# Lounes78/matcha-tts

Hardware: AMD Instinct MI355X
Metric: mel-frames/sec + RTF, text->wav @10 ODE steps, LJSpeech model, 1/2/4/8 GPU (higher is better)
Workload: dtype bf16

## Files before the change

include/matcha_hip.h:

```cpp
#ifndef MATCHA_HIP_H
#define MATCHA_HIP_H

#include <stddef.h>
#include <stdint.h>

#ifdef __cplusplus
extern "C" {
#endif

#define MT_DTYPE_F32 0
#define MT_DTYPE_BF16 1
#define MT_SOLVER_EULER 0
#define MT_SOLVER_MIDPOINT 1

const char* mt_last_error(void);
int mt_abi_version(void);
int mt_build_experiments(void);
int mt_sched_count(void);
int mt_sched_get(int i, int* rec, int* wait, int* wait_first, int cap);

typedef struct mt_encoder mt_encoder;
int mt_encoder_create(int n_vocab, int n_channels, int filter_channels, int n_heads, int n_layers, int kernel_size,
                      int n_spks, int spk_emb_dim, int dp_filter_channels, int dp_kernel_size, int prenet, int dtype,
                      mt_encoder** out);
// ... 176 lines not shown
                      int rows, int C, float* dx, void* stream);
int mtt_snake_fwd(const float* x, const float* log_alpha, const float* log_beta, size_t n, int C, float* y,
                  void* stream);
int mtt_snake_bwd(const float* x, const float* log_alpha, const float* log_beta, const float* dy, size_t n, int C,
                  float* dx, float* galpha, float* gbeta, void* stream);
int mtt_softmax_fwd(const float* s, const float* kmask, const float* qmask, int BH, int H, int Tq, int Tk, float scale,
                    int mode, float* p, void* stream);
int mtt_softmax_bwd(const float* p, const float* dp, const float* kmask, const float* qmask, int BH, int H, int Tq,
                    int Tk, float scale, float* ds, void* stream);
int mtt_rope(float* x, int B, int T, int H, int dh, int d, const float* theta, int inverse, void* stream);
int mtt_embed_fwd(const int64_t* ids, size_t ntok, const float* table, int C, float scale, float* out, void* stream);
int mtt_embed_bwd(const int64_t* ids, size_t ntok, const float* dout, int V, int C, float scale, float* dtable,
                  void* stream);
int mtt_adam(float* p, const float* g, float* m, float* v, size_t n, const float* gscale, float lr, float beta1,
             float beta2, float eps, int step, void* stream);
int mtt_clip_factor(const float* sumsq, float max_norm, float inv_world, float* out, float* norm_out, void* stream);
int mtt_unscale(float* g, size_t n, float inv_scale, float* found, float* scratch, void* stream);

size_t mt_op_conv1d_workspace_bytes(int dtype, int cin, int cout, int k, int stride, int transposed);
int mt_op_conv1d(int dtype, const void* x, int B, int Tin, int cin, const float* W, const float* bias,
                 int cout, int k, int stride, int pad, int dil, int transposed, float slope, void* y,
                 int Tout, void* ws, size_t ws_bytes, void* stream);
int mt_op_conv1d_tile(int variant, int dtype, const void* x, int B, int Tin, int cin, const float* W,
                      const float* bias, int cout, int k, int stride, int pad, int dil, int transposed,
                      float slope, void* y, int Tout, void* ws, size_t ws_bytes, void* stream);
size_t mt_op_vconv_workspace_bytes(int cin, int cout, int k);
int mt_op_vconv(const void* x, int B, int L, int cin, const float* W, const float* bias, int cout, int k, int dil,
                int ef, const void* resid, void* y, void* y2, float slope, float div, const int32_t* lens, int pack,
                void* ws, size_t ws_bytes, void* stream);
int mt_vconv_set_rbconv(int enable);
int mt_vconv_set_ct(int enable);
int mt_vpair_set_kernels(int mask);
int mt_vocoder_set_post_fold(int enable);
int mt_vconv_set_actin(int enable);
int mt_ffn_set(int enable);
int mt_ffn_set_min_frames(int frames);
int mt_decoder_set_kernels(int mask);
int mt_op_attention(int dtype, const void* qkv, const float* mask, void* out, int B, int T, int heads,
                    void* stream);

#define MT_PROBE_RBFUSE_C64 1
#define MT_PROBE_RBFUSE_C32 2
#define MT_PROBE_VCONV 3
#define MT_PROBE_VCONV_DEC 4
int mt_probe_start(int site, int max_launches);
int mt_probe_pause(int paused);
int mt_probe_detail(int cap, double* ms, double* flops, double* bytes, int* tags);
int mt_probe_stop(int* launches, double* total_ms, double* flops, double* bytes, double peak_flops, double peak_bw,
                  double* roof_ms);

#define MT_VCONV_LOG_FIELDS 11
int mt_vconv_log_start(int capacity);
int mt_vconv_log_stop(int32_t* records, int capacity);
int mt_vconv_log_select(int families);

#ifdef __cplusplus
}
#endif
#endif
```

matcha-tts_amd/csrc/mt_capi.hip:

```cpp
#include <string.h>

#include <new>

#include "../../include/matcha_hip.h"
#include "mt_ffn.h"
#include "mt_model.h"
#include "mt_vconv.h"
#include "mt_vpair.h"
#include "mt_probe.h"
#include "mt_train.h"

namespace mt {
const char* last_error();
int denoise(const float* audio, int B, int L, const float* bias_spec, float strength, float* out, void* ws,
            size_t ws_bytes, hipStream_t st, const int* lens = nullptr, int lmul = 1);
size_t denoise_workspace_bytes(int B, int L);
int vconv_exp_flags();
int rbconv_exp_flags();
int ffn_exp_flags();
int vpair_exp_flags();
int stft_magnitude(const float* audio, int B, int L, float* mag, hipStream_t st);
int log_mel(const float* audio, int B, int L, const float* basis, float mean, float stdv, float* mel, hipStream_t st);
size_t resample_workspace_bytes(int half, int up, int down);
int resample(const float* audio, int B, int L, const int* lens, int lmul, const float* taps, int half, int up,
// ... 19 lines not shown

struct mt_encoder {
  mt::Encoder e;
};
struct mt_decoder {
  mt::Decoder d;
};
struct mt_vocoder {
  mt::Vocoder v;
};

using mt::set_error;

static int param_name(const mt::ParamList& L, int i, char* buf, int buflen) {
  MT_REQUIRE(i >= 0 && i < (int)L.names.size(), "param index %d out of range", i);
  MT_REQUIRE(buf && buflen > (int)L.names[i].size(), "param name buffer too small");
  memcpy(buf, L.names[i].c_str(), L.names[i].size() + 1);
  return 0;
}
static int param_shape(const mt::ParamList& L, int i, int64_t* shape, int maxdim) {
  MT_REQUIRE(i >= 0 && i < (int)L.names.size(), "param index %d out of range", i);
  const auto& s = L.shapes[i];
  MT_REQUIRE((int)s.size() <= maxdim, "shape buffer too small");
  for (size_t k = 0; k < s.size(); ++k) shape[k] = s[k];
  return (int)s.size();
}

extern "C" {

const char* mt_last_error(void) { return mt::last_error(); }
int mt_abi_version(void) { return 1; }
int mt_vpair_set_kernels(int mask) { return mt::vpair_set_kernels(mask); }
int mt_vocoder_set_post_fold(int enable) { return mt::vocoder_set_post_fold(enable); }
int mt_sched_count(void) { return mt::sched_count(); }
int mt_sched_get(int i, int* rec, int* wait, int* wait_first, int cap) {
  MT_REQUIRE(rec && wait && wait_first, "null buffer");
  const int S = mt::sched_get(i, rec, wait, wait_first, cap);
  MT_REQUIRE(S >= 0, "schedule %d: out of range or cap %d too small", i, cap);
  return S;
}
int mt_build_experiments(void) {
  return (mt::vconv_exp_flags() ? 1 : 0) | (mt::rbconv_exp_flags() ? 2 : 0) | (mt::ffn_exp_flags() ? 4 : 0) |
         (mt::vpair_exp_flags() ? 8 : 0);
}

int mt_encoder_create(int n_vocab, int n_channels, int filter_channels, int n_heads, int n_layers, int kernel_size,
                      int n_spks, int spk_emb_dim, int dp_filter_channels, int dp_kernel_size, int prenet, int dtype,
                      mt_encoder** out) {
  MT_REQUIRE(out, "null out");
  mt_encoder* h = new (std::nothrow) mt_encoder();
  MT_REQUIRE(h, "out of host memory");
  int rc = h->e.init(n_vocab, n_channels, filter_channels, n_heads, n_layers, kernel_size, n_spks, spk_emb_dim,
                     dp_filter_channels, dp_kernel_size, prenet, dtype);
  if (rc) {
    delete h;
    return rc;
  }
  *out = h;
  return 0;
}
void mt_encoder_destroy(mt_encoder* e) { delete e; }
int mt_encoder_num_params(const mt_encoder* e) { return e ? (int)e->e.params.names.size() : -1; }
int mt_encoder_param_name(const mt_encoder* e, int i, char* buf, int buflen) {
  MT_REQUIRE(e, "null encoder");
  return param_name(e->e.params, i, buf, buflen);
}
// ... 609 lines not shown
```

matcha-tts_amd/csrc/mt_model.h:

```cpp
#pragma once
#include <memory>
#include <string>
#include <vector>

#include "mt_conv.h"
#include "mt_misc.h"
#include "mt_vconv.h"

namespace mt {

struct ParamList {
  std::vector<std::string> names;
  std::vector<std::vector<long long>> shapes;
  int add(const std::string& n, std::vector<long long> s) {
    names.push_back(n);
    shapes.push_back(std::move(s));
    return (int)names.size() - 1;
  }
};

struct Packer {
  size_t off = 0;
  size_t take(size_t bytes) {
    const size_t o = off;
// ... 160 lines not shown
  size_t emb_off = 0;
  struct Pre {
    GemmW conv;
    int g, b;
    size_t ln_off;
  };
  std::vector<Pre> pre;
  GemmW pre_proj;
  struct Layer {
    GemmW qkv, o, f1, f2;
    int n1g, n1b, n2g, n2b;
    size_t n1_off, n2_off;
    size_t s1_off = 0, s2_off = 0;
  };
  std::vector<Layer> lay;
  size_t ezero_off = 0;
  GemmW proj_m, dp1, dp2, dpp;
  int dn1g, dn1b, dn2g, dn2b, theta;
  size_t dn1_off, dn2_off, theta_off;

  int init(int n_vocab, int n_channels, int filter_channels, int heads, int layers, int kernel, int n_spks,
           int spk_dim, int dp_filter, int dp_kernel, int prenet, int dtype);
  int pack(const float* const* p, void* packed, hipStream_t st) const;
  size_t workspace_bytes(int B, int Tx) const;
  int forward(const void* packed, const long long* ids, const long long* xlen, const float* spks, int B, int Tx,
              float* mu, float* logw, float* xmask, int* oov, void* ws, size_t ws_bytes, hipStream_t st) const;
  template <class E>
  int forward_t(const char* P, const long long* ids, const long long* xlen, const float* spks, int B, int Tx,
                float* mu, float* logw, float* xmask, int* oov, char* ws, hipStream_t st) const;
};

int vocoder_post_fold();
int vocoder_set_post_fold(int enable);

struct Vocoder {
  int resblock = 1, dtype = BF16, esize = 2;
  int fuse = 1;
  int vconv = 2;
  int pair = 1;
  static constexpr int kDefaultWt = 0;
  int wt_stages = kDefaultWt;
  size_t zero_off = 0;
  bool any_vc = false;
  std::vector<int> up_rates, up_kernels, rb_kernels;
  std::vector<std::vector<int>> rb_dils;
  int up_init = 512, n_mels = 80;
  ParamList params;
  size_t packed_bytes = 0;
  GemmW pre, post;
  std::vector<GemmW> ups;
  std::vector<std::vector<GemmW>> rb1, rb2;

  int init(int resblock, const std::vector<int>& up_rates, const std::vector<int>& up_kernels, int up_init,
           const std::vector<int>& rb_kernels, const std::vector<std::vector<int>>& rb_dils, int dtype);
  int pack(const float* const* p, void* packed, hipStream_t st) const;
  bool stage_vc(int i) const;
  bool rb_vp(int i, int j) const;
  bool stage_vp(int i) const;
  bool stage_vp32(int i) const;
  int pair_resblock(const char* P, int i, int j, int B, int L, const char* X, char* XS, char* Tb, char* R,
                    char* RA, char* trash, bool act_out, hipStream_t st, const int* lens = nullptr,
                    float* wav = nullptr) const;
  int pair_chain(const char* P, int i, int B, int L, const char* X, char* XS, char* Tb, char* R, char* RA,
                 char* trash, bool act_out, hipStream_t st, const int* lens = nullptr, float* wav = nullptr) const;
  bool post_fold(int i) const;
  int rate_upto(int i) const;
// ... 18 lines not shown
```

matcha-tts_amd/csrc/mt_probe.cpp:

```cpp
#include "mt_probe.h"
#include "mt_vconv.h"

#include <algorithm>
#include <mutex>
#include <vector>

namespace mt {
namespace {
std::mutex g_mu;
int g_site = PROBE_NONE;
std::vector<hipEvent_t> g_ev;
int g_n = 0, g_cap = 0;
double g_flops = 0, g_bytes = 0;
std::vector<double> g_lf, g_lb;
std::vector<int> g_lt;
bool g_open = false;
bool g_paused = false;

void release() {
  for (hipEvent_t e : g_ev) (void)hipEventDestroy(e);
  g_ev.clear();
  g_n = g_cap = 0;
  g_flops = g_bytes = 0;
  g_lf.clear();
  g_lb.clear();
  g_lt.clear();
  g_site = PROBE_NONE;
  g_open = false;
  g_paused = false;
}
}

bool probe_armed(int site) { return g_site != PROBE_NONE && g_site == site; }
bool probe_any_armed() { return g_site != PROBE_NONE; }

void probe_begin(int site, hipStream_t st) {
  if (!probe_armed(site)) return;
  std::lock_guard<std::mutex> lk(g_mu);
  if (g_n >= g_cap || g_open || g_paused) return;
  (void)hipEventRecord(g_ev[2 * g_n], st);
  g_open = true;
}

void probe_end(int site, hipStream_t st, double flops, double bytes, int tag) {
  if (!probe_armed(site)) return;
  std::lock_guard<std::mutex> lk(g_mu);
  if (!g_open) return;
  (void)hipEventRecord(g_ev[2 * g_n + 1], st);
  g_open = false;
  ++g_n;
  g_flops += flops;
  g_bytes += bytes;
  g_lf.push_back(flops);
  g_lb.push_back(bytes);
  g_lt.push_back(tag);
}

int probe_detail(int cap, double* ms, double* flops, double* bytes, int* tags) {
  std::lock_guard<std::mutex> lk(g_mu);
  const int n = std::min(cap, g_n);
  for (int i = 0; i < n; ++i) {
    float t = 0.f;
    if (hipEventSynchronize(g_ev[2 * i + 1]) != hipSuccess ||
        hipEventElapsedTime(&t, g_ev[2 * i], g_ev[2 * i + 1]) != hipSuccess) {
      set_error("probe: event timing failed");
      return -1;
    }
    if (ms) ms[i] = t;
    if (flops) flops[i] = g_lf[i];
    if (bytes) bytes[i] = g_lb[i];
    if (tags) tags[i] = g_lt[i];
  }
  return n;
}

int probe_start(int site, int max_launches) {
  std::lock_guard<std::mutex> lk(g_mu);
  release();
  MT_REQUIRE(site > PROBE_NONE && site <= PROBE_VCONV_DEC, "probe: unknown site %d", site);
  MT_REQUIRE(max_launches > 0 && max_launches <= (1 << 16), "probe: max_launches %d", max_launches);
  g_ev.resize(2 * (size_t)max_launches);
  for (hipEvent_t& e : g_ev) MT_CHECK_HIP(hipEventCreate(&e));
  g_cap = max_launches;
  g_site = site;
  return 0;
}

int probe_pause(bool paused) {
  std::lock_guard<std::mutex> lk(g_mu);
  g_paused = paused;
  return 0;
}

int probe_stop(int* launches, double* total_ms, double* flops, double* bytes, double peak_flops, double peak_bw,
               double* roof_ms) {
  std::lock_guard<std::mutex> lk(g_mu);
  double ms = 0, roof = 0;
  for (int i = 0; i < g_n; ++i)
    roof += 1e3 * std::max(peak_flops > 0 ? g_lf[i] / peak_flops : 0.0, peak_bw > 0 ? g_lb[i] / peak_bw : 0.0);
  int rc = 0;
  for (int i = 0; i < g_n && rc == 0; ++i) {
    float t = 0.f;
    if (hipEventSynchronize(g_ev[2 * i + 1]) != hipSuccess ||
        hipEventElapsedTime(&t, g_ev[2 * i], g_ev[2 * i + 1]) != hipSuccess) {
      set_error("probe: event timing failed");
      rc = -1;
    }
    ms += t;
  }
  if (launches) *launches = g_n;
  if (total_ms) *total_ms = ms;
  if (flops) *flops = g_flops;
  if (bytes) *bytes = g_bytes;
  if (roof_ms) *roof_ms = roof;
  release();
  return rc;
}

namespace {
std::vector<int> g_log;
int g_log_cap = 0;
bool g_log_on = false;
}

namespace {
struct SchedEntry {
  int rec[SCHED_FIELDS];
  SchedWaits waits;
};
std::vector<SchedEntry>& sched_table() {
  static std::vector<SchedEntry> t;
  return t;
}
}

int sched_register(const int (&rec)[SCHED_FIELDS], SchedWaits waits) {
  auto& t = sched_table();
  for (const auto& e : t)
    if (std::equal(e.rec, e.rec + SCHED_FIELDS, rec)) return 0;
  SchedEntry e;
  std::copy(rec, rec + SCHED_FIELDS, e.rec);
  e.waits = waits;
  t.push_back(e);
// ... 49 lines not shown
```

matcha-tts_amd/csrc/mt_probe.h:

```cpp
#pragma once
#include "mt_common.h"

namespace mt {

enum ProbeSite {
  PROBE_NONE = 0,
  PROBE_RBFUSE_C64 = 1,
  PROBE_RBFUSE_C32 = 2,
  PROBE_VCONV = 3,
  PROBE_VCONV_DEC = 4,
};

bool probe_armed(int site);
bool probe_any_armed();
void probe_begin(int site, hipStream_t st);
enum ProbeTag { PROBE_TAG_VCONV = 0, PROBE_TAG_VPAIR = 1, PROBE_TAG_VPAIR32 = 2, PROBE_TAG_RBFUSE = 3, PROBE_TAG_VPAIR128 = 4, PROBE_TAG_RBCONV = 5 };
void probe_end(int site, hipStream_t st, double flops, double bytes, int tag = PROBE_TAG_VCONV);
int probe_detail(int cap, double* ms, double* flops, double* bytes, int* tags);
int probe_start(int site, int max_launches);
int probe_pause(bool paused);
int probe_stop(int* launches, double* total_ms, double* flops, double* bytes, double peak_flops, double peak_bw,
               double* roof_ms);

constexpr int VCLOG_FIELDS = 11;
enum : int { VCLOG_CONV = 1, VCLOG_AUX = 2 };
void vclog_record(const int (&rec)[VCLOG_FIELDS], int family = VCLOG_CONV);
int vclog_select(int families);
int vclog_start(int cap);
int vclog_stop(int* out, int cap);
bool vclog_armed();

}
```

matcha-tts_amd/csrc/mt_vocoder.hip:

```cpp
#include <algorithm>
#include <type_traits>

#include "mt_model.h"
#include "mt_ragged.h"
#include "mt_rbfuse.h"
#include "mt_vconv.h"
#include "mt_vpair.h"

namespace mt {

constexpr int PC_N = 256;
__global__ __launch_bounds__(256) void post_conv_kernel(const bf16* __restrict__ x, int L,
                                                        const bf16* __restrict__ w, const float* __restrict__ bias,
                                                        float slope, float* __restrict__ out, const int* lens,
                                                        int lmul) {
  __shared__ __attribute__((aligned(16))) char rows[(PC_N + 16) * 64];
  const int b = blockIdx.y, f0 = blockIdx.x * PC_N, tid = threadIdx.x, lane = tid & 63, wave = tid >> 6;
  const bf16* xb = x + (size_t)b * L * 32;
  const int Lb = lens ? min(max(lens[b] * lmul, 0), L) : L;
  if (f0 >= Lb) {
    if (f0 + tid < L) out[(size_t)b * L + f0 + tid] = 0.f;
    return;
  }
  for (int e = tid; e < (PC_N + 6) * 4; e += 256) {
// ... 215 lines not shown
}

bool Vocoder::stage_vp32(int i) const {
  const int nk = (int)rb_kernels.size();
  if (!pair || !fuse || vconv < 2 || !any_vc || dtype != BF16 || resblock != 1 || rb1[(size_t)i * nk].empty()) return false;
  for (int j = 0; j < nk; ++j)
    for (size_t q = 0; q < rb1[(size_t)i * nk + j].size(); ++q) {
      const GemmW& a = rb1[(size_t)i * nk + j][q];
      const GemmW& b = rb2[(size_t)i * nk + j][q];
      for (const GemmW* g : {&a, &b})
        if (g->cin != 32 || g->cout != 32 || g->Mpad != 32 || g->cin_pad != 32 || g->taps != g->k) return false;
      if (!vpair32_supported(a.k, a.dil) || b.k != a.k || b.dil != 1) return false;
    }
  return true;
}

static int g_postfold = -1;
int vocoder_post_fold() {
  if (g_postfold < 0) {
    const char* e = getenv("MT_POSTFOLD");
    g_postfold = e && e[0] == '0' ? 0 : 1;
  }
  return g_postfold;
}
int vocoder_set_post_fold(int enable) {
  const int prev = vocoder_post_fold();
  g_postfold = enable ? 1 : 0;
  return prev;
}

bool Vocoder::post_fold(int i) const {
  const int nk = (int)rb_kernels.size();
  return vocoder_post_fold() && dtype == BF16 && i + 1 == (int)ups.size() && stage_vp32(i) && post.cin == 32 &&
         post.k == 7 && post.cout == 1 && nk > 0 && (rb_kernels[nk - 1] - 1) / 2 <= 5;
}

int Vocoder::pair_resblock(const char* P, int i, int j, int B, int L, const char* X, char* XS, char* Tb, char* R,
                           char* RA, char* trash, bool act_out, hipStream_t st, const int* lens, float* wav) const {
  const int nk = (int)rb_kernels.size();
  const int C = rb1[(size_t)i * nk][0].cout;
  const bool c32 = C == 32;
  int rc;
  const std::vector<GemmW>& c1 = rb1[(size_t)i * nk + j];
  const std::vector<GemmW>& c2 = rb2[(size_t)i * nk + j];
  const int np = (int)c1.size();
  const char* state = X;
  for (int q = 0; q < np; ++q) {
    const bool last = q == np - 1;
    VPairArgs a{};
    a.x = (const bf16*)state;
    a.B = B;
    a.L = L;
    a.w1 = (const bf16*)(P + (c32 ? c1[q].w_off : c1[q].v_off));
    a.b1 = (const float*)(P + c1[q].b_off);
    a.w2 = (const bf16*)(P + (c32 ? c2[q].w_off : c2[q].v_off));
    a.b2 = (const float*)(P + c2[q].b_off);
    a.taps = c1[q].k;
    a.dil = c1[q].dil;
    a.div = (float)nk;
    a.slope = 0.1f;
    a.zero = (const bf16*)(P + zero_off);
    a.trash = (bf16*)trash;
    a.lens = lens;
    a.lmul = rate_upto(i + 1);
    int ef = 0;
    if (!last) {
      a.y = (bf16*)((q & 1) ? Tb : R);
    } else {
      a.y = (bf16*)XS;
      if (j > 0) ef |= VE_ACCUM;
      if (j == nk - 1) ef |= VE_DIV;
      if (j == nk - 1 && act_out) {
        a.y2 = (bf16*)RA;
        ef |= VE_DUAL | VE_Y2ONLY;
      }
      if (j == nk - 1 && wav && c32 && !act_out && j > 0) {
        a.post_w = (const bf16*)(P + post.w_off);
        a.post_b = (const float*)(P + post.b_off);
        a.post_slope = 0.01f;
// ... 371 lines not shown
```

matcha-tts_amd/csrc/mt_vpair.h:

```cpp
#pragma once
#include <algorithm>

#include "mt_probe.h"
#include "mt_ragged.h"
#include "mt_vconv.h"

namespace mt {

struct VPairArgs {
  const bf16* x;
  int B, L;
  const bf16* w1;
  const float* b1;
  const bf16* w2;
  const float* b2;
  int taps, dil;
  bf16* y;
  bf16* y2;
  float div, slope;
  const bf16* zero;
  bf16* trash;
  const int* lens;
  int lmul;
  const bf16* post_w;
// ... 156 lines not shown
      return (OPT & VE_POST) != 0;
  }
#undef MT_PAIR_EF
  return false;
}

template <class F>
int pair_launch(const char* name, int C, int bn, int ef, const VPairArgs& a, hipStream_t st, int tag, F&& launch) {
  const long ntiles = (long)a.B * ((a.L + bn - 1) / bn);
  MT_REQUIRE(ntiles < (1L << 31), "%s: too many tiles", name);
  const int G = (int)std::min<long>(ntiles, cu_count());
  const double flops = 2.0 * 2.0 * C * C * a.taps * (double)a.B * a.L;
  const double bytes = 2.0 * (2.0 * 2.0 * C * (double)a.B * a.L) + 2.0 * 2.0 * C * C * a.taps;
  probe_begin(PROBE_VCONV, st);
  if (!launch(G)) {
    set_error("%s: epilogue %d not compiled in", name, ef);
    return -1;
  }
  MT_CHECK_HIP(hipGetLastError());
  probe_end(PROBE_VCONV, st, flops, bytes, tag);
  const int rec[VCLOG_FIELDS] = {ef | 0x10000, C, bn, 0, (int)ntiles, G, a.taps, C, C, a.B, a.L};
  vclog_record(rec);
  return 0;
}

enum : int { VPK_CTK = 1, VPK_CTK128 = 2, VPK_ALL = 3 };
int vpair_kernels();
int vpair_set_kernels(int mask);

bool vpair_supported(int C, int k, int d);
int launch_vpair(int ef, const VPairArgs& a, hipStream_t st);
bool vpair32_supported(int k, int d);
int launch_vpair32(int ef, const VPairArgs& a, hipStream_t st);
bool vpair128_supported(int k, int d);
int launch_vpair128(int ef, const VPairArgs& a, hipStream_t st);

}
```

matcha-tts_amd/csrc/mt_vpair32.hip:

```cpp
#include <algorithm>
#include <type_traits>

#include "mt_probe.h"
#include "mt_ts.h"
#include "mt_vpair.h"

namespace mt {

namespace {
constexpr int NT = 512, C = 32;
constexpr int FN = 6;
constexpr int WNC = 16 * FN;
constexpr int NF1 = 8 * WNC;
constexpr int HALO2 = 8;
constexpr int BN = NF1 - 2 * HALO2;
constexpr int RB = C * 2;
constexpr int XROWS = NF1 + 128;
constexpr int XBUF = XROWS * RB;
constexpr int TROWS = NF1 + 16;
constexpr int TBUF = TROWS * RB;
constexpr int KMAX = 11;
constexpr int TAPW = C * RB;
constexpr int T_OFF = XBUF, W_OFF = T_OFF + TBUF, PAR_OFF = W_OFF + 2 * KMAX * TAPW;
constexpr int RAG_OFF = PAR_OFF + 2 * C * 4;
// ... 261 lines not shown
      }
    }
    issued += POST ? 2 : FN * ((EF & VE_DUAL) ? 2 : 1);
    VP_TS(9);
  }
  asm volatile("s_waitcnt vmcnt(0)" ::: "memory");
  VP_TS(11);
  VP_TS_END(wave, lane);
}

bool vpair32_supported(int k, int d) {
  return k >= 3 && k % 2 == 1 && k <= KMAX && (k - 1) / 2 <= HALO2 && NF1 + d * (k - 1) <= XROWS;
}

int launch_vpair32(int ef, const VPairArgs& a, hipStream_t st) {
  ef &= ~VE_Y2ONLY;
  if (pair_check("vpair32", ef, a, vpair32_supported(a.taps, a.dil) && a.taps % 2 == 1)) return -1;
  MT_REQUIRE(!(ef & VE_POST) || (a.post_w && a.post_b && a.wav && (ef & ~VE_POST) == (VE_ACCUM | VE_DIV) &&
                                 (a.taps - 1) / 2 + 3 <= HALO2),
             "vpair32: VE_POST needs conv_post's weights, bias and the waveform, the stage's final (ACCUM | DIV) pair "
             "and k <= %d", 2 * (HALO2 - 3) + 1);
  const bool wt = store_policy() == ST_WT;
  return pair_launch("vpair32", C, BN, ef, a, st, PROBE_TAG_VPAIR32, [&](int G) {
    return pair_with_ef<VE_POST>(ef, [&](auto ec) {
      constexpr int E = decltype(ec)::value;
      if constexpr ((E & VE_POST) != 0)
        hipLaunchKernelGGL((vpair32_kernel<E>), dim3(G), dim3(NT), 0, st, a);
      else if (wt) hipLaunchKernelGGL((vpair32_kernel<E, ST_WT>), dim3(G), dim3(NT), 0, st, a);
      else hipLaunchKernelGGL((vpair32_kernel<E>), dim3(G), dim3(NT), 0, st, a);
    });
  });
}

VP_TS_BINDER(vpair32_ts_bind)

}
```

matcha-tts_amd/matcha_hip/_lib.py:

```python
from __future__ import annotations

import ctypes
import os
from ctypes import POINTER, c_char_p, c_double, c_float, c_int, c_int64, c_size_t, c_uint, c_void_p

PKG_DIR = os.path.dirname(os.path.dirname(os.path.abspath(__file__)))
LIB_PATH = os.path.join(PKG_DIR, "libmatcha_hip.so")

DTYPE_F32 = 0
DTYPE_BF16 = 1
SOLVER_EULER = 0
SOLVER_MIDPOINT = 1

P = c_void_p

SIGNATURES = {
    "mt_last_error": (c_char_p, []),
    "mt_abi_version": (c_int, []),
    "mt_build_experiments": (c_int, []),
    "mt_sched_count": (c_int, []),
    "mt_sched_get": (c_int, [c_int, P, P, P, c_int]),
    "mt_encoder_create": (c_int, [c_int, c_int, c_int, c_int, c_int, c_int, c_int, c_int, c_int, c_int, c_int, c_int,
                                  POINTER(c_void_p)]),
    "mt_encoder_destroy": (None, [P]),
# ... 60 lines not shown
    "mt_denoise": (c_int, [P, c_int, c_int, P, c_float, P, P, c_size_t, P]),
    "mt_denoise_ragged": (c_int, [P, c_int, c_int, P, c_int, P, c_float, P, P, c_size_t, P]),
    "mt_resample_workspace_bytes": (c_size_t, [c_int, c_int, c_int]),
    "mt_resample": (c_int, [P, c_int, c_int, P, c_int, P, c_int, c_int, c_int, P, c_int, P, P, c_size_t, P]),
    "mt_resample_range": (c_int, [P, c_int, c_int, P, c_int, P, c_int, c_int, c_int, c_int, c_int, P, P, P, c_size_t,
                                  P]),
    "mt_window_gather": (c_int, [P, c_int, c_int, c_int, P, P, P, c_int, c_int, P, P]),
    "mt_window_scatter": (c_int, [P, c_int, c_int, P, P, P, P, P, c_int, c_int, P]),
    "mt_audio_stats_workspace_bytes": (c_size_t, [c_int, c_int]),
    "mt_audio_stats": (c_int, [P, c_int, c_int, P, P, P, P, c_size_t, P]),
    "mt_audio_encode": (c_int, [P, c_int, c_int, P, P, P, c_int, c_double, c_int, c_int, P, P, P]),
    "mt_loudness_workspace_bytes": (c_size_t, [c_int, c_int, c_int]),
    "mt_loudness": (c_int, [P, c_int, c_int, P, POINTER(c_double), c_int, c_double, P, c_int, P, P, P, c_size_t, P]),
    "mt_true_peak_workspace_bytes": (c_size_t, [c_int, c_int]),
    "mt_true_peak": (c_int, [P, c_int, c_int, P, P, c_int, P, P, P, c_size_t, P]),
    "mt_maximum_path_workspace_bytes": (c_size_t, [c_int, c_int, c_int]),
    "mt_decoder_step_times_workspace_bytes": (c_size_t, [P, c_int, c_int]),
    "mt_decoder_step_times": (c_int, [P, P, P, P, P, P, P, c_int, c_int, P, P, c_size_t, P]),
    "mt_maximum_path": (c_int, [P, P, P, c_int, c_int, c_int, P, P, c_size_t, P]),
    "mt_stft_magnitude": (c_int, [P, c_int, c_int, P, P]),
    "mt_log_mel": (c_int, [P, c_int, c_int, P, c_float, c_float, P, P]),
    "mt_op_conv1d_workspace_bytes": (c_size_t, [c_int, c_int, c_int, c_int, c_int, c_int]),
    "mt_op_conv1d": (c_int, [c_int, P, c_int, c_int, c_int, P, P, c_int, c_int, c_int, c_int, c_int,
                             c_int, c_float, P, c_int, P, c_size_t, P]),
    "mt_op_conv1d_tile": (c_int, [c_int, c_int, P, c_int, c_int, c_int, P, P, c_int, c_int, c_int, c_int, c_int,
                                  c_int, c_float, P, c_int, P, c_size_t, P]),
    "mt_op_vconv_workspace_bytes": (c_size_t, [c_int, c_int, c_int]),
    "mt_op_vconv": (c_int, [P, c_int, c_int, c_int, P, P, c_int, c_int, c_int, c_int, P, P, P, c_float, c_float,
                            P, c_int, P, c_size_t, P]),
    "mt_vconv_set_rbconv": (c_int, [c_int]),
    "mt_vconv_set_ct": (c_int, [c_int]),
    "mt_vpair_set_kernels": (c_int, [c_int]),
    "mt_vocoder_set_post_fold": (c_int, [c_int]),
    "mt_ffn_set": (c_int, [c_int]),
    "mt_vconv_set_actin": (c_int, [c_int]),
    "mt_ffn_set_min_frames": (c_int, [c_int]),
    "mt_decoder_set_kernels": (c_int, [c_int]),
    "mt_op_attention": (c_int, [c_int, P, P, P, c_int, c_int, c_int, P]),
    "mt_probe_start": (c_int, [c_int, c_int]),
    "mt_probe_pause": (c_int, [c_int]),
    "mt_probe_detail": (c_int, [c_int, P, P, P, P]),
    "mt_probe_stop": (c_int, [P, P, P, P, c_double, c_double, P]),
    "mtt_gemm": (c_int, [c_int, c_int, c_int, c_int, c_int, c_float, P, c_int, c_int64, P, c_int, c_int64, c_float,
                         P, c_int, c_int64, c_int, P, P, P, c_size_t, P]),
    "mtt_gemm_ex": (c_int, [c_int, c_int, c_int, c_int, c_int, c_int, c_float, P, c_int, c_int64, P, c_int, c_int64,
                            c_float, P, c_int, c_int64, c_int, P, P, P, c_size_t, P]),
    "mtt_gemm_workspace_bytes": (c_size_t, [c_int, c_int, c_int, c_int]),
    "mtt_im2col": (c_int, [P, P, c_int, c_int, c_int, c_int, c_int, c_int, c_int, c_int, P, P]),
    "mtt_col2im": (c_int, [P, P, c_int, c_int, c_int, c_int, c_int, c_int, c_int, c_int, P, c_int, P]),
    "mtt_ew": (c_int, [c_int, c_size_t, P, P, P, P, c_float, c_float, c_size_t, c_size_t, c_size_t, c_size_t,
                       c_size_t, c_size_t, c_int, P]),
    "mtt_copy_cols": (c_int, [P, c_int, c_int, P, c_int, c_int, c_int, c_int, c_int, P]),
    "mtt_seq_mask": (c_int, [P, c_int, c_int, P, P]),
    "mtt_colsum_scratch_floats": (c_size_t, [c_int, c_int, c_int]),
    "mtt_colsum": (c_int, [P, P, c_int, c_int, c_int, P, c_int, P, P]),
    "mtt_bcast_cols": (c_int, [P, c_int, P, c_int, c_int, c_int, c_int, P]),
    "mtt_segsum_cols_scratch_floats": (c_size_t, [c_int, c_int, c_int]),
    "mtt_segsum_cols": (c_int, [P, c_int, c_int, c_int, c_int, c_int, P, c_int, P, P]),
    "mtt_sum": (c_int, [P, P, c_size_t, P, P, P]),
    "mtt_dropout": (c_int, [P, c_size_t, c_float, c_uint, P, P]),
    "mtt_groupnorm_fwd": (c_int, [P, P, P, c_int, c_int, c_int, c_int, c_float, P, P, P, P]),
    "mtt_groupnorm_bwd": (c_int, [P, P, P, P, P, c_int, c_int, c_int, c_int, P, P, P, P]),
    "mtt_layernorm_fwd": (c_int, [P, P, P, c_int, c_int, c_float, P, P, P, P]),
    "mtt_layernorm_bwd": (c_int, [P, P, P, P, P, c_int, c_int, P, P]),
    "mtt_snake_fwd": (c_int, [P, P, P, c_size_t, c_int, P, P]),
    "mtt_snake_bwd": (c_int, [P, P, P, P, c_size_t, c_int, P, P, P, P]),
# ... 62 lines not shown
```

matcha-tts_amd/matcha_hip/runtime.py:

```python
from __future__ import annotations

import math
import numbers
import time
from ctypes import byref, c_char_p, c_double, c_int, c_int32, c_int64, c_void_p, create_string_buffer
from typing import Dict, List, Optional, Tuple

import torch

from ._lib import (DTYPE_BF16, DTYPE_F32, SOLVER_EULER, SOLVER_MIDPOINT, HipPathError, check, lib,
                   ptr, stream_handle)

_DTYPES = {"fp32": DTYPE_F32, "float32": DTYPE_F32, "f32": DTYPE_F32,
           "bf16": DTYPE_BF16, "bfloat16": DTYPE_BF16,
           "fp32x3": DTYPE_F32}


def dtype_code(precision: str) -> int:
    try:
        return _DTYPES[precision]
    except KeyError:
        raise ValueError(f"precision must be one of {sorted(set(_DTYPES))}, got {precision!r}")


# ... 991 lines not shown
    if y is None:
        y = torch.empty((B, L, cout), dtype=torch.bfloat16, device=x.device)
    if (ef & 16) and y2 is None:
        y2 = torch.empty((B, L, cout), dtype=torch.bfloat16, device=x.device)
    if resid is not None:
        resid = resid.to(torch.bfloat16).contiguous()
    L_ = lib()
    nb = L_.mt_op_vconv_workspace_bytes(cin, cout, k)
    if ws is None or ws.numel() < nb:
        if not pack:
            raise ValueError("op_vconv: pack=False needs the workspace a packing call filled")
        ws = torch.empty(nb, dtype=torch.uint8, device=x.device)
    W, bias = f32c(W), f32c(bias)
    if lens is not None:
        lens = lens.to(device=x.device, dtype=torch.int32).contiguous()
    check(L_.mt_op_vconv(ptr(x), B, L, cin, ptr(W), ptr(bias), cout, k, dil, int(ef), ptr(resid), ptr(y), ptr(y2),
                         float(slope), float(div), ptr(lens), int(bool(pack)), ws.data_ptr(), ws.numel(),
                         stream_handle(x.device)), "op_vconv")
    return y, y2


def set_vconv_ct(enable: bool) -> bool:
    return bool(lib().mt_vconv_set_ct(int(bool(enable))))


def set_vpair_kernels(mask: int) -> int:
    return int(lib().mt_vpair_set_kernels(int(mask)))


def set_post_fold(enable) -> int:
    return int(lib().mt_vocoder_set_post_fold(int(bool(enable))))


def set_ffn(mode) -> int:
    return int(lib().mt_ffn_set(int(mode)))


def set_ffn_min_frames(frames: int) -> int:
    return int(lib().mt_ffn_set_min_frames(int(frames)))


def set_decoder_kernels(mask: int) -> int:
    return int(lib().mt_decoder_set_kernels(int(mask)))


def set_rbconv_actin(enable: bool) -> bool:
    return bool(lib().mt_vconv_set_actin(int(bool(enable))))


def set_rbconv(enable: bool) -> bool:
    return bool(lib().mt_vconv_set_rbconv(int(bool(enable))))


def op_attention(qkv: torch.Tensor, mask: torch.Tensor, heads: int, precision="fp32") -> torch.Tensor:
    require_gpu(qkv, mask, what="op_attention")
    dt = dtype_code(precision)
    et = torch.bfloat16 if dt == DTYPE_BF16 else torch.float32
    qkv = qkv.to(et).contiguous()
    B, T, _ = qkv.shape
    out = torch.empty((B, T, heads * 64), dtype=et, device=qkv.device)
    mask = f32c(mask.reshape(B, T))
    check(lib().mt_op_attention(dt, ptr(qkv), ptr(mask), ptr(out), B, T, heads, stream_handle(qkv.device)),
          "op_attention")
    return out


# ... 53 lines not shown
```

Baseline: 825,800.

## Fuse a whole 32-channel vocoder ResBlock's three conv pairs into one kernel

Adds a vrb32 kernel that runs all three dilated k=3 conv pairs of a 32-channel HiFi-GAN ResBlock in a single launch. The intermediate activations and residual stay in LDS across the pairs, using a 16-frame halo that is recomputed at tile edges. The fused path is on by default (MT_RBFUSE env) whenever the block qualifies, and it cuts two launches plus the global round-trips between pairs. In exchange it recomputes halo frames, uses a large LDS footprint that may lower occupancy, and adds a post_fold guard change and probe accounting for the multi-part launches.

Result: no change. 831,700, median of 6 (+0.7%).

```diff
diff --git a/include/matcha_hip.h b/include/matcha_hip.h
--- a/include/matcha_hip.h
+++ b/include/matcha_hip.h
@@ -232,6 +232,8 @@
 int mt_vconv_set_ct(int enable);
 int mt_vpair_set_kernels(int mask);
 int mt_vocoder_set_post_fold(int enable);
+int mt_vocoder_set_rb_fuse(int enable);
+int mt_vocoder_rb_fusable(int dtype, int channels, int npairs, int k, const int* dils, int ef);
 int mt_vconv_set_actin(int enable);
 int mt_ffn_set(int enable);
 int mt_ffn_set_min_frames(int frames);
diff --git a/matcha-tts_amd/csrc/mt_capi.hip b/matcha-tts_amd/csrc/mt_capi.hip
--- a/matcha-tts_amd/csrc/mt_capi.hip
+++ b/matcha-tts_amd/csrc/mt_capi.hip
@@ -75,6 +75,10 @@
 int mt_abi_version(void) { return 1; }
 int mt_vpair_set_kernels(int mask) { return mt::vpair_set_kernels(mask); }
 int mt_vocoder_set_post_fold(int enable) { return mt::vocoder_set_post_fold(enable); }
+int mt_vocoder_set_rb_fuse(int enable) { return mt::vocoder_set_rb_fuse(enable); }
+int mt_vocoder_rb_fusable(int dtype, int channels, int npairs, int k, const int* dils, int ef) {
+  return mt::vrb32_fusable(dtype == mt::BF16, channels, npairs, k, dils, ef) ? 1 : 0;
+}
 int mt_sched_count(void) { return mt::sched_count(); }
 int mt_sched_get(int i, int* rec, int* wait, int* wait_first, int cap) {
   MT_REQUIRE(rec && wait && wait_first, "null buffer");
diff --git a/matcha-tts_amd/csrc/mt_model.h b/matcha-tts_amd/csrc/mt_model.h
--- a/matcha-tts_amd/csrc/mt_model.h
+++ b/matcha-tts_amd/csrc/mt_model.h
@@ -216,6 +216,8 @@
 
 int vocoder_post_fold();
 int vocoder_set_post_fold(int enable);
+int vocoder_rb_fuse();
+int vocoder_set_rb_fuse(int enable);
 
 struct Vocoder {
   int resblock = 1, dtype = BF16, esize = 2;
diff --git a/matcha-tts_amd/csrc/mt_probe.cpp b/matcha-tts_amd/csrc/mt_probe.cpp
--- a/matcha-tts_amd/csrc/mt_probe.cpp
+++ b/matcha-tts_amd/csrc/mt_probe.cpp
@@ -14,6 +14,7 @@
 double g_flops = 0, g_bytes = 0;
 std::vector<double> g_lf, g_lb;
 std::vector<int> g_lt;
+std::vector<int> g_lp;
 bool g_open = false;
 bool g_paused = false;
 
@@ -25,6 +26,7 @@
   g_lf.clear();
   g_lb.clear();
   g_lt.clear();
+  g_lp.clear();
   g_site = PROBE_NONE;
   g_open = false;
   g_paused = false;
@@ -42,7 +44,7 @@
   g_open = true;
 }
 
-void probe_end(int site, hipStream_t st, double flops, double bytes, int tag) {
+void probe_end(int site, hipStream_t st, double flops, double bytes, int tag, int parts) {
   if (!probe_armed(site)) return;
   std::lock_guard<std::mutex> lk(g_mu);
   if (!g_open) return;
@@ -54,22 +56,26 @@
   g_lf.push_back(flops);
   g_lb.push_back(bytes);
   g_lt.push_back(tag);
+  g_lp.push_back(std::max(parts, 1));
 }
 
 int probe_detail(int cap, double* ms, double* flops, double* bytes, int* tags) {
   std::lock_guard<std::mutex> lk(g_mu);
-  const int n = std::min(cap, g_n);
-  for (int i = 0; i < n; ++i) {
+  int n = 0;
+  for (int i = 0; i < g_n && n < cap; ++i) {
     float t = 0.f;
     if (hipEventSynchronize(g_ev[2 * i + 1]) != hipSuccess ||
         hipEventElapsedTime(&t, g_ev[2 * i], g_ev[2 * i + 1]) != hipSuccess) {
       set_error("probe: event timing failed");
       return -1;
     }
-    if (ms) ms[i] = t;
-    if (flops) flops[i] = g_lf[i];
-    if (bytes) bytes[i] = g_lb[i];
-    if (tags) tags[i] = g_lt[i];
+    const int parts = g_lp[i];
+    for (int p = 0; p < parts && n < cap; ++p, ++n) {
+      if (ms) ms[n] = t / parts;
+      if (flops) flops[n] = g_lf[i] / parts;
+      if (bytes) bytes[n] = g_lb[i] / parts;
+      if (tags) tags[n] = g_lt[i];
+    }
   }
   return n;
 }
@@ -108,7 +114,9 @@
     }
     ms += t;
   }
-  if (launches) *launches = g_n;
+  int entries = 0;
+  for (int i = 0; i < g_n; ++i) entries += g_lp[i];
+  if (launches) *launches = entries;
   if (total_ms) *total_ms = ms;
   if (flops) *flops = g_flops;
   if (bytes) *bytes = g_bytes;
diff --git a/matcha-tts_amd/csrc/mt_probe.h b/matcha-tts_amd/csrc/mt_probe.h
--- a/matcha-tts_amd/csrc/mt_probe.h
+++ b/matcha-tts_amd/csrc/mt_probe.h
@@ -15,7 +15,7 @@
 bool probe_any_armed();
 void probe_begin(int site, hipStream_t st);
 enum ProbeTag { PROBE_TAG_VCONV = 0, PROBE_TAG_VPAIR = 1, PROBE_TAG_VPAIR32 = 2, PROBE_TAG_RBFUSE = 3, PROBE_TAG_VPAIR128 = 4, PROBE_TAG_RBCONV = 5 };
-void probe_end(int site, hipStream_t st, double flops, double bytes, int tag = PROBE_TAG_VCONV);
+void probe_end(int site, hipStream_t st, double flops, double bytes, int tag = PROBE_TAG_VCONV, int parts = 1);
 int probe_detail(int cap, double* ms, double* flops, double* bytes, int* tags);
 int probe_start(int site, int max_launches);
 int probe_pause(bool paused);
diff --git a/matcha-tts_amd/csrc/mt_vocoder.hip b/matcha-tts_amd/csrc/mt_vocoder.hip
--- a/matcha-tts_amd/csrc/mt_vocoder.hip
+++ b/matcha-tts_amd/csrc/mt_vocoder.hip
@@ -271,7 +271,21 @@
 bool Vocoder::post_fold(int i) const {
   const int nk = (int)rb_kernels.size();
   return vocoder_post_fold() && dtype == BF16 && i + 1 == (int)ups.size() && stage_vp32(i) && post.cin == 32 &&
-         post.k == 7 && post.cout == 1 && nk > 0 && (rb_kernels[nk - 1] - 1) / 2 <= 5;
+         post.k == 7 && post.cout == 1 && nk >= 2 && (rb_kernels[nk - 1] - 1) / 2 <= 5;
+}
+
+static int g_rbfuse = -1;
+int vocoder_rb_fuse() {
+  if (g_rbfuse < 0) {
+    const char* e = getenv("MT_RBFUSE");
+    g_rbfuse = e && e[0] == '0' ? 0 : 1;
+  }
+  return g_rbfuse;
+}
+int vocoder_set_rb_fuse(int enable) {
+  const int prev = vocoder_rb_fuse();
+  g_rbfuse = enable ? 1 : 0;
+  return prev;
 }
 
 int Vocoder::pair_resblock(const char* P, int i, int j, int B, int L, const char* X, char* XS, char* Tb, char* R,
@@ -284,6 +298,41 @@
   const std::vector<GemmW>& c2 = rb2[(size_t)i * nk + j];
   const int np = (int)c1.size();
   const char* state = X;
+  if (c32 && np == VRB_NP && vocoder_rb_fuse()) {
+    int ef = (j > 0 ? VE_ACCUM : 0) | (j == nk - 1 ? VE_DIV : 0);
+    if (j == nk - 1 && act_out) ef |= VE_DUAL | VE_Y2ONLY;
+    if (j == nk - 1 && wav && !act_out && j > 0) ef |= VE_POST;
+    int dils[VRB_NP];
+    bool k3 = true;
+    for (int q = 0; q < np; ++q) {
+      dils[q] = c1[q].dil;
+      k3 = k3 && c1[q].k == 3 && c2[q].k == 3 && c2[q].dil == 1;
+    }
+    if (k3 && vrb32_fusable(dtype == BF16, C, np, 3, dils, ef)) {
+      VRb32Args a{};
+      a.p.x = (const bf16*)X;
+      a.p.B = B;
+      a.p.L = L;
+      a.p.taps = 3;
+      a.p.dil = dils[0];
+      a.p.y = (bf16*)XS;
+      a.p.div = (float)nk;
+      a.p.slope = 0.1f;
+      a.p.zero = (const bf16*)(P + zero_off);
+      a.p.trash = (bf16*)trash;
+      a.p.lens = lens;
+      a.p.lmul = rate_upto(i + 1);
+      for (int q = 0; q < np; ++q) {
+        a.w1[q] = (const bf16*)(P + c1[q].w_off);
+        a.b1[q] = (const float*)(P + c1[q].b_off);
+        a.w2[q] = (const bf16*)(P + c2[q].w_off);
+        a.b2[q] = (const float*)(P + c2[q].b_off);
+        a.dil[q] = dils[q];
+      }
+      a.p.w1 = a.w1[0], a.p.b1 = a.b1[0], a.p.w2 = a.w2[0], a.p.b2 = a.b2[0];
+      return launch_vrb32(ef, a, st);
+    }
+  }
   for (int q = 0; q < np; ++q) {
     const bool last = q == np - 1;
     VPairArgs a{};
diff --git a/matcha-tts_amd/csrc/mt_vpair.h b/matcha-tts_amd/csrc/mt_vpair.h
--- a/matcha-tts_amd/csrc/mt_vpair.h
+++ b/matcha-tts_amd/csrc/mt_vpair.h
@@ -212,6 +212,16 @@
 int launch_vpair(int ef, const VPairArgs& a, hipStream_t st);
 bool vpair32_supported(int k, int d);
 int launch_vpair32(int ef, const VPairArgs& a, hipStream_t st);
+constexpr int VRB_NP = 3;
+struct VRb32Args {
+  VPairArgs p;
+  const bf16 *w1[VRB_NP], *w2[VRB_NP];
+  const float *b1[VRB_NP], *b2[VRB_NP];
+  int dil[VRB_NP];
+};
+enum : int { VCLOG_RB = 1 << 22, VCLOG_RB_HEAD = 1 << 23 };
+bool vrb32_fusable(bool is_bf16, int C, int npairs, int k, const int* dils, int ef);
+int launch_vrb32(int ef, const VRb32Args& a, hipStream_t st);
 bool vpair128_supported(int k, int d);
 int launch_vpair128(int ef, const VPairArgs& a, hipStream_t st);
 
diff --git a/matcha-tts_amd/csrc/mt_vpair32.hip b/matcha-tts_amd/csrc/mt_vpair32.hip
--- a/matcha-tts_amd/csrc/mt_vpair32.hip
+++ b/matcha-tts_amd/csrc/mt_vpair32.hip
@@ -317,6 +317,325 @@
   });
 }
 
+namespace {
+constexpr int RB_K = 3;
+constexpr int RB_HALO = 16;
+constexpr int RB_BN = NF1 - 2 * RB_HALO;
+constexpr int RB_MS = 16;
+constexpr int RB_ROWS = NF1 + 2 * RB_MS;
+constexpr int RB_PIECES = RB_ROWS / 16;
+constexpr int RB_BUF = RB_ROWS * RB;
+constexpr int RB_NCONV = 2 * VRB_NP;
+constexpr int RB_T_OFF = RB_BUF, RB_W_OFF = 2 * RB_BUF, RB_PAR_OFF = RB_W_OFF + RB_NCONV * RB_K * TAPW;
+constexpr int RB_RAG_OFF = RB_PAR_OFF + RB_NCONV * C * 4;
+constexpr int RB_LDS_BYTES = RB_RAG_OFF + RAG_LDS;
+static_assert(RB_LDS_BYTES <= 160 * 1024, "LDS budget");
+static_assert(RB_NCONV * RB_K * TAPW <= 2 * KMAX * TAPW, "the six convs' weights fit the pair kernel's weight area");
+static_assert(RB_HALO % 16 == 0 && RB_BN == 8 * WNC - 2 * RB_HALO && RB_BN % 16 == 0, "whole fragments discarded");
+static_assert(RB_HALO >= (1 + 1) + (3 + 1) + (5 + 1), "the v1 dilations' accumulated halo");
+static_assert(RB_ROWS % 16 == 0 && RB_PIECES <= 7 * 8, "row staging: at most 7 pieces per wave");
+static_assert(RB_MS + NF1 - 1 + RB_MS < RB_ROWS && RB_W_OFF % 1024 == 0, "tap reads stay inside the row buffers");
+}
+
+bool vrb32_fusable(bool is_bf16, int Cn, int npairs, int k, const int* dils, int ef) {
+  if (!is_bf16 || Cn != C || npairs != VRB_NP || k != RB_K || !dils) return false;
+  ef &= ~VE_Y2ONLY;
+  if (ef != 0 && ef != VE_ACCUM && ef != (VE_ACCUM | VE_DIV)) return false;
+  int h = 0;
+  for (int q = 0; q < VRB_NP; ++q) {
+    if (dils[q] < 1 || dils[q] > RB_MS) return false;
+    h += dils[q] + 1;
+  }
+  return h <= RB_HALO;
+}
+
+template <int EF, int SP = ST_PLAIN>
+__global__ __launch_bounds__(NT) void vrb32_kernel(VRb32Args a) {
+  static_assert(!(EF & (VE_POST | VE_DUAL)), "VE_POST / VE_DUAL stay on per-pair launches");
+  static_assert(SP == ST_PLAIN || VP32_BUF, "the store policy rides on the 16-byte buffer stores");
+  __shared__ __attribute__((aligned(1024))) char smem[RB_LDS_BYTES];
+  const int tid = threadIdx.x, lane = tid & 63;
+  const int wave = __builtin_amdgcn_readfirstlane(tid >> 6);
+  const int g4 = lane >> 4, l16 = lane & 15, lrow = lane >> 2, lp = lane & 3;
+  const int L = a.p.L;
+  const float slope = a.p.slope;
+  PairWalk tiles;
+  if (!tiles.init(a.p, smem + RB_RAG_OFF, RB_BN, tid)) return;
+  const int nmine = tiles.nmine;
+  if (tid < C) {
+    float* pw = reinterpret_cast<float*>(smem + RB_PAR_OFF);
+#pragma unroll
+    for (int q = 0; q < VRB_NP; ++q) {
+      pw[(2 * q) * C + tid] = a.b1[q][tid];
+      pw[(2 * q + 1) * C + tid] = a.b2[q][tid];
+    }
+  }
+  __syncthreads();
+
+  int issued = 0, xmk = 0;
+  RagTile nxt;
+  auto stage_weights = [&]() {
+    for (int j = wave; j < 2 * RB_K * RB_NCONV; j += 8) {
+      const int cv = j / (2 * RB_K), t = (j >> 1) - cv * RB_K, r = (j & 1) * 16 + lrow;
+      const bf16* w = a.w1[0];
+#pragma unroll
+      for (int q = 0; q < VRB_NP; ++q) {
+        if (cv == 2 * q) w = a.w1[q];
+        if (cv == 2 * q + 1) w = a.w2[q];
+      }
+      glds16(w + ((size_t)r * RB_K + t) * C + (lp ^ swz(r)) * 8, smem + RB_W_OFF + (cv * RB_K + t) * TAPW + (j & 1) * 1024);
+      ++issued;
+    }
+  };
+  const int xlane = lrow * RB + ((lp ^ swz(lrow)) * 16);
+  const int npiece = (RB_PIECES - wave + 7) / 8;
+  auto stage_x = [&](int ti) __attribute__((always_inline)) {
+    nxt = tiles.at(ti);
+    if constexpr (VP32_BUF) {
+      const int b = __builtin_amdgcn_readfirstlane(nxt.b);
+      const int f0 = __builtin_amdgcn_readfirstlane(nxt.n0 - RB_HALO - RB_MS);
+      const unsigned nrec = ti < nmine ? (unsigned)__builtin_amdgcn_readfirstlane(nxt.lv) * RB : 0u;
+      const auto xr = __builtin_amdgcn_make_buffer_rsrc(const_cast<bf16*>(a.p.x + (size_t)b * L * C), (short)0, (int)nrec,
+                                                        0x00020000);
+#pragma unroll
+      for (int i = 0; i < 7; ++i) {
+        const int j = wave + 8 * i;
+        if (j < RB_PIECES)
+          __builtin_amdgcn_raw_ptr_buffer_load_lds(xr, (__attribute__((address_space(3))) void*)(smem + j * 1024), 16,
+                                                   (unsigned)(xlane + (f0 + 16 * j) * RB), 0, 0, 0);
+      }
+    } else {
+      const bool live = ti < nmine;
+      const bf16* xb = a.p.x + (size_t)(live ? nxt.b : 0) * L * C;
+      const int f0 = nxt.n0 - RB_HALO - RB_MS, lv = nxt.lv;
+#pragma unroll
+      for (int i = 0; i < 7; ++i) {
+        const int j = wave + 8 * i;
+        if (j < RB_PIECES) {
+          const int r = 16 * j + lrow;
+          const int q = lp ^ swz(r);
+          const int f = f0 + r;
+          const bool ok = live && f >= 0 && f < lv;
+          glds16(ok ? xb + (size_t)f * C + q * 8 : a.p.zero + q * 8, smem + j * 1024);
+        }
+      }
+    }
+    issued += npiece;
+    xmk = issued;
+  };
+
+  auto conv_epi = [&](int cv, const char* src, int rb0, int tstride, auto&& epi) __attribute__((always_inline)) {
+    bf16x8 A[RB_K][2], Bf[2][RB_K];
+#pragma unroll
+    for (int t = 0; t < RB_K; ++t)
+#pragma unroll
+      for (int f = 0; f < 2; ++f)
+        A[t][f] = *reinterpret_cast<const bf16x8*>(smem + RB_W_OFF + (cv * RB_K + t) * TAPW + (l16 + f * 16) * RB +
+                                                   ((g4 ^ swz(l16)) * 16));
+    auto read_b = [&](bf16x8(&B)[RB_K], int fn) __attribute__((always_inline)) {
+#pragma unroll
+      for (int t = 0; t < RB_K; ++t) {
+        const int rb = rb0 + t * tstride + fn * 16;
+        B[t] = *reinterpret_cast<const bf16x8*>(src + rb * RB + ((g4 ^ swz(rb)) * 16));
+      }
+    };
+    read_b(Bf[0], 0);
+#pragma unroll
+    for (int fn = 0; fn < FN; ++fn) {
+      if (fn + 1 < FN) read_b(Bf[(fn + 1) & 1], fn + 1);
+      f32x4 acc0 = mfma16(A[0][0], Bf[fn & 1][0], f32x4{0.f, 0.f, 0.f, 0.f});
+      f32x4 acc1 = mfma16(A[0][1], Bf[fn & 1][0], f32x4{0.f, 0.f, 0.f, 0.f});
+#pragma unroll
+      for (int t = 1; t < RB_K; ++t) {
+        acc0 = mfma16(A[t][0], Bf[fn & 1][t], acc0);
+        acc1 = mfma16(A[t][1], Bf[fn & 1][t], acc1);
+      }
+      epi(fn, acc0, acc1);
+    }
+  };
+
+  stage_weights();
+  stage_x(0);
+
+  const float* par = reinterpret_cast<const float*>(smem + RB_PAR_OFF);
+  const int ch16 = (g4 & 1) * 16 + (g4 >> 1) * 8;
+  const int qc = (g4 & 1) * 2 + (g4 >> 1);
+  VP_TS_DECL
+  for (int ti = 0; ti < nmine; ++ti) {
+    const int b = nxt.b, n0 = nxt.n0;
+    const int Lt = nxt.lv;
+    VP_TS(10);
+    wait_vmcnt(issued - xmk);
+    VP_TS(0);
+    lds_barrier();
+    VP_TS(1);
+    uint32_t res[FN][2][2];
+    u32x4 yv[FN];
+#pragma unroll
+    for (int fn = 0; fn < FN; ++fn) {
+      const int r = RB_MS + wave * WNC + fn * 16 + l16;
+      unpack16(*reinterpret_cast<const u32x4*>(smem + r * RB + ((qc ^ swz(r)) * 16)), res[fn]);
+    }
+    lds_barrier();
+    VP_TS(2);
+#pragma unroll
+    for (int i = 0; i < (RB_BUF / 16 + NT - 1) / NT; ++i) {
+      const int e = tid + i * NT;
+      if (e < RB_BUF / 16) {
+        u32x4 v = *reinterpret_cast<const u32x4*>(smem + e * 16);
+#pragma unroll
+        for (int w = 0; w < 4; ++w) v[w] = lrelu_pk(v[w], slope);
+        *reinterpret_cast<u32x4*>(smem + e * 16) = v;
+      }
+    }
+    lds_barrier();
+    VP_TS(3);
+    int ymk = 0;
+    const int bu = __builtin_amdgcn_readfirstlane(b);
+#pragma unroll
+    for (int q = 0; q < VRB_NP; ++q) {
+      const int dq = a.dil[q];
+      const bool lastp = q == VRB_NP - 1;
+      if constexpr ((EF & VE_ACCUM) != 0) {
+        if (lastp) {
+#pragma unroll
+          for (int fn = 0; fn < FN; ++fn) {
+            const int i = min(max(n0 - RB_HALO + wave * WNC + fn * 16 + l16, 0), L - 1);
+            asm volatile("global_load_dwordx4 %0, %1, off"
+                         : "=v"(yv[fn])
+                         : "v"(a.p.y + ((size_t)b * L + i) * C + ch16)
+                         : "memory");
+          }
+          issued += FN;
+          ymk = issued;
+        }
+      }
+      {
+        const f32x4 bA = *reinterpret_cast<const f32x4*>(par + (2 * q) * C + 4 * g4);
+        const f32x4 bB = *reinterpret_cast<const f32x4*>(par + (2 * q) * C + 16 + 4 * g4);
+        conv_epi(2 * q, smem, wave * WNC + l16 + RB_MS - dq, dq, [&](int fn, const f32x4& a0, const f32x4& a1) {
+          const int j = wave * WNC + fn * 16 + l16;
+          const int f = n0 - RB_HALO + j;
+          const bool ok = f >= 0 && f < Lt;
+          uint32_t o[2][2];
+          o[0][0] = ok ? lrelu_pk_f(f32x2{a0[0], a0[1]} + f32x2{bA[0], bA[1]}, slope) : 0u;
+          o[0][1] = ok ? lrelu_pk_f(f32x2{a0[2], a0[3]} + f32x2{bA[2], bA[3]}, slope) : 0u;
+          o[1][0] = ok ? lrelu_pk_f(f32x2{a1[0], a1[1]} + f32x2{bB[0], bB[1]}, slope) : 0u;
+          o[1][1] = ok ? lrelu_pk_f(f32x2{a1[2], a1[3]} + f32x2{bB[2], bB[3]}, slope) : 0u;
+          const int r = RB_MS + j;
+          *reinterpret_cast<u32x4*>(smem + RB_T_OFF + r * RB + ((qc ^ swz(r)) * 16)) = pack16(o);
+        });
+      }
+      VP_TS(4);
+      lds_barrier();
+      if (lastp) stage_x(ti + 1);
+      VP_TS(6);
+      const f32x4 bA = *reinterpret_cast<const f32x4*>(par + (2 * q + 1) * C + 4 * g4);
+      const f32x4 bB = *reinterpret_cast<const f32x4*>(par + (2 * q + 1) * C + 16 + 4 * g4);
+      const int rb2 = wave * WNC + l16 + RB_MS - 1;
+      if (!lastp) {
+        conv_epi(2 * q + 1, smem + RB_T_OFF, rb2, 1, [&](int fn, const f32x4& a0, const f32x4& a1) {
+          const int j = wave * WNC + fn * 16 + l16;
+          const int f = n0 - RB_HALO + j;
+          const bool ok = f >= 0 && f < Lt;
+          uint32_t o2[2][2];
+#pragma unroll
+          for (int h = 0; h < 2; ++h) {
+            const f32x4& ac = h ? a1 : a0;
+            const f32x4& b4 = h ? bB : bA;
+#pragma unroll
+            for (int u = 0; u < 2; ++u) {
+              uint32_t o1;
+              res_out<VE_RESID>(f32x2{ac[2 * u], ac[2 * u + 1]}, f32x2{b4[2 * u], b4[2 * u + 1]}, res[fn][h][u], 0u,
+                                a.p.div, slope, o1, o2[h][u]);
+              res[fn][h][u] = ok ? o1 : 0u;
+              o2[h][u] = ok ? o2[h][u] : 0u;
+            }
+          }
+          const int r = RB_MS + j;
+          *reinterpret_cast<u32x4*>(smem + r * RB + ((qc ^ swz(r)) * 16)) = pack16(o2);
+        });
+        VP_TS(7);
+        lds_barrier();
+        VP_TS(8);
+        continue;
+      }
+      if constexpr ((EF & VE_ACCUM) != 0) {
+        wait_vmcnt(issued - ymk);
+#pragma unroll
+        for (int fn = 0; fn < FN; ++fn) asm volatile("" : "+v"(yv[fn]));
+      }
+      VP_TS(8);
+      const auto yr = __builtin_amdgcn_make_buffer_rsrc(a.p.y + (size_t)bu * L * C, (short)0, (int)((unsigned)L * RB), 0x00020000);
+      conv_epi(2 * q + 1, smem + RB_T_OFF, rb2, 1, [&](int fn, const f32x4& a0, const f32x4& a1) {
+        const int j = wave * WNC + fn * 16 + l16;
+        uint32_t yy[2][2] = {}, o1[2][2], o2[2][2];
+        if constexpr ((EF & VE_ACCUM) != 0) unpack16(yv[fn], yy);
+#pragma unroll
+        for (int h = 0; h < 2; ++h) {
+          const f32x4& ac = h ? a1 : a0;
+          const f32x4& b4 = h ? bB : bA;
+#pragma unroll
+          for (int u = 0; u < 2; ++u) {
+            res_out<EF | VE_RESID>(f32x2{ac[2 * u], ac[2 * u + 1]}, f32x2{b4[2 * u], b4[2 * u + 1]}, res[fn][h][u],
+                                   yy[h][u], a.p.div, slope, o1[h][u], o2[h][u]);
+          }
+        }
+        const u32x4 y = pack16(o1);
+        const bool keep = !(fn == 0 && wave == 0) && !(fn == FN - 1 && wave == 7);
+        if constexpr (VP32_BUF) {
+          const unsigned vo = keep ? (unsigned)(((n0 - RB_HALO + j) * C + ch16) * 2) : 0x80000000u;
+          buf_store16<SP>(y, yr, vo);
+        } else {
+          const bool ok = keep && n0 - RB_HALO + j < L;
+          const size_t o = ((size_t)b * L + n0 - RB_HALO + j) * C + ch16;
+          *reinterpret_cast<u32x4*>(ok ? a.p.y + o : a.p.trash + 8 * lane) = y;
+        }
+      });
+      issued += FN;
+      VP_TS(7);
+    }
+  }
+  asm volatile("s_waitcnt vmcnt(0)" ::: "memory");
+  VP_TS(11);
+  VP_TS_END(wave, lane);
+}
+
+int launch_vrb32(int ef, const VRb32Args& a, hipStream_t st) {
+  ef &= ~VE_Y2ONLY;
+  if (pair_check("vrb32", ef, a.p, a.p.taps == RB_K)) return -1;
+  MT_REQUIRE(vrb32_fusable(true, C, VRB_NP, a.p.taps, a.dil, ef),
+             "vrb32: k %d, dilations %d %d %d, epilogue %d: not a fusable ResBlock", a.p.taps, a.dil[0], a.dil[1],
+             a.dil[2], ef);
+  for (int q = 0; q < VRB_NP; ++q) MT_REQUIRE(a.w1[q] && a.w2[q] && a.b1[q] && a.b2[q], "vrb32: null weights (pair %d)", q);
+  const bool wt = store_policy() == ST_WT;
+  const long ntiles = (long)a.p.B * ((a.p.L + RB_BN - 1) / RB_BN);
+  MT_REQUIRE(ntiles < (1L << 31), "vrb32: too many tiles");
+  const int G = (int)std::min<long>(ntiles, cu_count());
+  const double flops = VRB_NP * (2.0 * 2.0 * C * C * RB_K * (double)a.p.B * a.p.L);
+  const double bytes = VRB_NP * (2.0 * (2.0 * 2.0 * C * (double)a.p.B * a.p.L) + 2.0 * 2.0 * C * C * RB_K);
+  probe_begin(PROBE_VCONV, st);
+  const bool known = pair_with_ef<0>(ef, [&](auto ec) {
+    constexpr int E = decltype(ec)::value;
+    if constexpr (E == 0 || E == VE_ACCUM || E == (VE_ACCUM | VE_DIV)) {
+      if (wt) hipLaunchKernelGGL((vrb32_kernel<E, ST_WT>), dim3(G), dim3(NT), 0, st, a);
+      else hipLaunchKernelGGL((vrb32_kernel<E>), dim3(G), dim3(NT), 0, st, a);
+    }
+  });
+  if (!known) {
+    set_error("vrb32: epilogue %d not compiled in", ef);
+    return -1;
+  }
+  MT_CHECK_HIP(hipGetLastError());
+  probe_end(PROBE_VCONV, st, flops, bytes, PROBE_TAG_VPAIR32, VRB_NP);
+  for (int q = 0; q < VRB_NP; ++q) {
+    const int e = (q == VRB_NP - 1 ? ef : 0) | 0x10000 | VCLOG_RB | (q == 0 ? VCLOG_RB_HEAD : 0);
+    const int rec[VCLOG_FIELDS] = {e, C, RB_BN, 0, (int)ntiles, G, RB_K, C, C, a.p.B, a.p.L};
+    vclog_record(rec);
+  }
+  return 0;
+}
+
 VP_TS_BINDER(vpair32_ts_bind)
 
 }
diff --git a/matcha-tts_amd/matcha_hip/_lib.py b/matcha-tts_amd/matcha_hip/_lib.py
--- a/matcha-tts_amd/matcha_hip/_lib.py
+++ b/matcha-tts_amd/matcha_hip/_lib.py
@@ -116,6 +116,8 @@
     "mt_vconv_set_ct": (c_int, [c_int]),
     "mt_vpair_set_kernels": (c_int, [c_int]),
     "mt_vocoder_set_post_fold": (c_int, [c_int]),
+    "mt_vocoder_set_rb_fuse": (c_int, [c_int]),
+    "mt_vocoder_rb_fusable": (c_int, [c_int, c_int, c_int, c_int, P, c_int]),
     "mt_ffn_set": (c_int, [c_int]),
     "mt_vconv_set_actin": (c_int, [c_int]),
     "mt_ffn_set_min_frames": (c_int, [c_int]),
diff --git a/matcha-tts_amd/matcha_hip/runtime.py b/matcha-tts_amd/matcha_hip/runtime.py
--- a/matcha-tts_amd/matcha_hip/runtime.py
+++ b/matcha-tts_amd/matcha_hip/runtime.py
@@ -1047,6 +1047,19 @@
     return int(lib().mt_vocoder_set_post_fold(int(bool(enable))))
 
 
+def set_rb_fuse(enable) -> int:
+    return int(lib().mt_vocoder_set_rb_fuse(int(bool(enable))))
+
+
+VCLOG_RB, VCLOG_RB_HEAD = 1 << 22, 1 << 23
+
+
+def rb_fusable(dtype: int, channels: int, npairs: int, k: int, dils, ef: int) -> bool:
+    import ctypes
+    arr = (ctypes.c_int * max(len(dils), 1))(*[int(d) for d in dils])
+    return bool(lib().mt_vocoder_rb_fusable(int(dtype), int(channels), int(npairs), int(k), arr, int(ef)))
+
+
 def set_ffn(mode) -> int:
     return int(lib().mt_ffn_set(int(mode)))
 
```
